# Algorithmic-Alignment-Lab/sco_py

Hardware: AMD Instinct MI355X
Metric: SCO iters/sec (batch of N trajopt QPs) (higher is better)
Workload: dtype f64

## Files before the change

include/sco_hip.h:

```cpp
#ifndef SCO_HIP_H
#define SCO_HIP_H

#ifdef __cplusplus
extern "C" {
#endif

#define SCO_OK              0
#define SCO_ERR_ARG        -1
#define SCO_ERR_DEVICE     -2
#define SCO_ERR_NO_GPU     -3
#define SCO_ERR_STATE      -4
#define SCO_ERR_CAPACITY   -5

#define SCO_QP_SOLVED                 1
#define SCO_QP_SOLVED_INACCURATE      2
#define SCO_QP_MAX_ITER_REACHED      -2
#define SCO_QP_PRIMAL_INFEASIBLE     -3
#define SCO_QP_PRIMAL_INFEASIBLE_INACCURATE 3
#define SCO_QP_DUAL_INFEASIBLE       -4
#define SCO_QP_DUAL_INFEASIBLE_INACCURATE   4
#define SCO_QP_NON_CVX               -7
#define SCO_QP_UNSOLVED             -10

const char *sco_last_error(void);
// ... 159 lines not shown

int sco_sqp_solve(sco_sqp *h, const sco_sqp_params *params, const sco_qp_settings *qp_settings);

int sco_sqp_fetch(sco_sqp *h, double *x, int *success, int *sqp_iters, int *qp_solves,
                  long long *admm_iters, double *merit, double *max_violation);

#define SCO_SQP_FLAG_MEMO_FULL 1
#define SCO_SQP_FLAG_CAPPED 2
#define SCO_SQP_FLAG_TRACE_FULL 4
int sco_sqp_fetch_flags(sco_sqp *h, int *flags);
int sco_sqp_last_rounds(const sco_sqp *h, int *rounds);
int sco_sqp_last_launches(const sco_sqp *h, int *launches, int *groups);

int sco_sqp_last_tiers(const sco_sqp *h, double ms[2], long long iters[2], int launches[2]);

int sco_debug_sqp_mixed(const sco_sqp *h, int out[2]);
int sco_debug_mix_split(int live, int cus, int xcds, int slack, int per_cu);

int sco_debug_wv_gres_slot(int nstep, int pos, int out[5]);

int sco_debug_sqp_schedule(const int in[12], int plan[20], const int round_in[3], int round_out[8]);
int sco_debug_stage_sweep(int n, const double *begin_ms, const double *end_ms, const int *stage, double ms[5]);

int sco_debug_sqp_layout(const sco_trajopt_desc *desc, int n_rows, const int *row_ptr, const int *col_idx, const int *row_is_eq,
                         int dims[22], int sizes[15], int *ints, double *vals);
int sco_debug_sqp_check_program(const sco_trajopt_desc *desc, int n_circle_rows, int n_words, const int *words, const int *row_ptr,
                                int n_consts, int n_params);

int sco_debug_qp_launch_plan(const int *in, const double *tol, int *out);
int sco_debug_plan_tiers(int *mask);

int sco_debug_lanes(int device, int op, const double *a, const double *b, double *out_a, double *out_b);

int sco_sqp_trace(sco_sqp *h, int cap, double *trace, int *n_entries);

int sco_sqp_last_timing(const sco_sqp *h, double ms[5]);

#ifdef __cplusplus
}
#endif
#endif
```

sco_py_amd/_lib.py:

```python
import ctypes as C
import os

import numpy as np

from . import _build

SCO_OK = 0
ERR_NAMES = {-1: "SCO_ERR_ARG", -2: "SCO_ERR_DEVICE", -3: "SCO_ERR_NO_GPU",
             -4: "SCO_ERR_STATE", -5: "SCO_ERR_CAPACITY"}


class ScoHipError(RuntimeError):
    def __init__(self, code, msg):
        super().__init__("%s (%d): %s" % (ERR_NAMES.get(code, "SCO_ERR"), code, msg))
        self.code = code


class QpSettings(C.Structure):
    _fields_ = [
        ("rho", C.c_double), ("sigma", C.c_double), ("alpha", C.c_double),
        ("eps_abs", C.c_double), ("eps_rel", C.c_double),
        ("eps_prim_inf", C.c_double), ("eps_dual_inf", C.c_double),
        ("max_iter", C.c_int), ("check_termination", C.c_int), ("scaling", C.c_int),
        ("warm_start", C.c_int), ("adaptive_rho", C.c_int), ("adaptive_rho_interval", C.c_int),
# ... 54 lines not shown
    "sco_sqp_load_quadratic": (C.c_int, [C.c_void_p, _DP, _DP, _DP]),
    "sco_sqp_load_spatial": (C.c_int, [C.c_void_p, _DP, _DP, _DP, _DP, _DP]),
    "sco_sqp_load_program": (C.c_int, [C.c_void_p, C.c_int, _IP, _IP, C.c_int, _DP, C.c_int, _DP]),
    "sco_sqp_load_program_steps": (C.c_int, [C.c_void_p, C.c_int, _IP, _IP, C.c_int, _DP, C.c_int, _DP]),
    "sco_sqp_load_obj_weights": (C.c_int, [C.c_void_p, _DP]),
    "sco_sqp_load_acc_weights": (C.c_int, [C.c_void_p, _DP]),
    "sco_sqp_load_linear_rows": (C.c_int, [C.c_void_p, _DP, _DP]),
    "sco_sqp_set_circle_rows": (C.c_int, [C.c_void_p, C.c_int]),
    "sco_sqp_load_vel_limit": (C.c_int, [C.c_void_p, _DP]),
    "sco_sqp_load_joint_limits": (C.c_int, [C.c_void_p, _DP, _DP]),
    "sco_sqp_load_ee_cost": (C.c_int, [C.c_void_p, _DP, _DP]),
    "sco_sqp_set_groups": (C.c_int, [C.c_void_p, C.c_int, C.POINTER(C.c_uint)]),
    "sco_sqp_fetch_groups": (C.c_int, [C.c_void_p, C.POINTER(C.c_uint)]),
    "sco_sqp_fetch_stalled_groups": (C.c_int, [C.c_void_p, C.POINTER(C.c_uint)]),
    "sco_sqp_fetch_flags": (C.c_int, [C.c_void_p, _IP]),
    "sco_sqp_last_rounds": (C.c_int, [C.c_void_p, _IP]),
    "sco_sqp_last_launches": (C.c_int, [C.c_void_p, _IP, _IP]),
    "sco_sqp_last_tiers": (C.c_int, [C.c_void_p, _DP, _LP, _IP]),
    "sco_debug_sqp_mixed": (C.c_int, [C.c_void_p, _IP]),
    "sco_debug_mix_split": (C.c_int, [C.c_int, C.c_int, C.c_int, C.c_int, C.c_int]),
    "sco_debug_wv_gres_slot": (C.c_int, [C.c_int, C.c_int, _IP]),
    "sco_debug_sqp_schedule": (C.c_int, [_IP, _IP, _IP, _IP]),
    "sco_debug_stage_sweep": (C.c_int, [C.c_int, _DP, _DP, _IP, _DP]),
    "sco_debug_sqp_layout": (C.c_int, [C.POINTER(TrajoptDesc), C.c_int, _IP, _IP, _IP, _IP, _IP, _IP, _DP]),
    "sco_debug_sqp_check_program": (C.c_int, [C.POINTER(TrajoptDesc), C.c_int, C.c_int, _IP, _IP, C.c_int, C.c_int]),
    "sco_debug_qp_launch_plan": (C.c_int, [_IP, _DP, _IP]),
    "sco_debug_plan_tiers": (C.c_int, [_IP]),
    "sco_debug_lanes": (C.c_int, [C.c_int, C.c_int, _DP, _DP, _DP, _DP]),
    "sco_sqp_solve": (C.c_int, [C.c_void_p, C.POINTER(SqpParams), C.POINTER(QpSettings)]),
    "sco_sqp_fetch": (C.c_int, [C.c_void_p, _DP, _IP, _IP, _IP, _LP, _DP, _DP]),
    "sco_sqp_trace": (C.c_int, [C.c_void_p, C.c_int, _DP, _IP]),
    "sco_sqp_last_timing": (C.c_int, [C.c_void_p, _DP]),
}

_lib = None


def lib_path():
    return _build.LIB


def load():
    global _lib
    if _lib is not None:
        return _lib
    path = lib_path()
# ... 141 lines not shown
```

sco_py_amd/csrc/sco_sqp.hip:

```cpp
#include "sco_admm_check.h"
#include "sqp_layout.h"
#include "sqp_rows.h"
#include "sqp_sched.h"

#include <algorithm>

#include <cmath>
#include <cstdio>
#include <cstdlib>
#include <cstring>

enum { ST_PROJECT = 0, ST_CONVEXIFY = 1, ST_TRIAL = 2, ST_DONE = 3 };
enum { STEP_PROJECT = 0, STEP_ACCEPT = 1, STEP_SHRINK = 2, STEP_YCONV = 3, STEP_XCONV = 4, STEP_BAD = 5, STEP_GROUP = 6 };

#define TRACE_W 8

struct SqpScalars {
  double penalty, trust, slack_cost, merit, merit_viol;
  long long admm_iters;
  int state, k, sqp_iters, qp_solves, success, escalations, n_trace, spawned;
  int flags;
};

struct EventPool {
// ... 42 lines not shown
  int *newqp;
  const int *list;
  int *list_buf;
  const int *jpos;
  const int *epos;
  int G;
  const unsigned int *gmask;
  const unsigned int *goverlap;
  double *mvec;
  unsigned int *nonconv;
  unsigned int *stalled;
  int H, HC;
  double *hkey, *hval, *ckey, *cJ, *cb;
  int *hn, *cn;
};

struct sco_sqp {
  int device = 0;
  sco_trajopt_desc desc{};
  sco_qp *qp0 = nullptr, *qp1 = nullptr;
  SqpDev d{};
  hipStream_t stream = nullptr;
  hipStream_t gstream[SQP_MAX_GROUPS - 1] = {};
  EventPool events, gevents[SQP_MAX_GROUPS];
  EventPool done{{}, 0, hipEventDisableTiming};
  EventPool mix_events{{}, 0, hipEventDisableTiming};
  int xcds = 0;
  double *fetch_buf = nullptr;
  int *host_active = nullptr;
  int groups_used = 1;
  std::vector<void *> allocs;
  void *prog_buf[4] = {nullptr, nullptr, nullptr, nullptr};
  void *objw_buf = nullptr;
  void *accw_buf = nullptr;
  bool gen_loaded = false;
  size_t prog_bytes[4] = {0, 0, 0, 0};
  bool loaded = false, solved = false, target_loaded = false, vel_loaded = false, jl_loaded = false, cost_loaded = false, quad_loaded = false, prog_loaded = false, spatial_loaded = false;
  double last_ms[5] = {0, 0, 0, 0, 0};
  int rounds = 0;
  int launches = 0;
  int wv_rounds = 0;
  double wv_ms = 0.0;
  int mixed_rounds = 0, mixed_side = 0;
};

__device__ __forceinline__ int memo_find(const double *keys, int count, int d, const double *x) {
// ... 264 lines not shown
          }
          wave_lds_fence();
        }
    double lam = A[0];
    for (int i = 1; i < n; i++) lam = fmin(lam, A[i * WIDE_LD + i]);
    if (lane < n) {
      if (lam < 0.0) Ht[lane * n + lane] -= lam;
      const double g = oA[t * n + lane];
      double acc = 0.0;
      for (int i = 0; i < n; i++) acc += th[i] * Ht[i * n + lane];
      xh[lane] = acc; gl[lane] = g;
      oA[t * n + lane] = g - acc;
    }
    wave_lds_fence();
    if (lane == 0) {
      double xHx = 0.0, gx = 0.0;
      for (int j = 0; j < n; j++) { xHx += xh[j] * th[j]; gx += gl[j] * th[j]; }
      ob[t] = (0.5 * xHx - gx) + of0[t];
    }
    wave_lds_fence();
  }
}

template <bool WIDE>
__device__ __forceinline__ void sqp_pre_body(SqpDev &s, QpDev &q1, SqpParamsDev &p) {
  const int g = blockIdx.x + s.b0, tid = threadIdx.x;
  const int b = s.list ? s.list[g] : g;
  if (b < 0) return;
  SqpScalars &sc = s.sc[b];
  const int state = sc.state;
  const bool parked = q1.prog && q1.prog[b] > 0;
  if (tid == 0) s.newqp[b] = (state != ST_DONE && !parked) ? 1 : 0;
  if (state == ST_DONE || parked) return;
  __shared__ double red[NWAVE * 4];
  __shared__ double of0[260];
  const int n_x = s.n_x, d = s.d, T = s.T, R = s.R, n = s.n, m = s.m;
  const int ds = s.ds, NBt = s.NBt;
  const int NO = s.cost == OBJ_BLOCK ? NBt : T;
  const RowLay L{T, NBt, R, s.Req};
  double *x = s.x + (size_t)b * n_x, *xs = s.x_saved + (size_t)b * n_x;
  double *gs = s.gsave + (size_t)b * s.m_nl, *J = s.J + (size_t)b * s.m_nl * ds, *bm = s.bmod + (size_t)b * s.m_nl;
  unsigned char *mask = s.mask + (size_t)b * s.m_nl * ds;
  const double penalty = sc.penalty, trust = sc.trust;
  const int spawned = sc.spawned;
  int k_rows = sc.k;
  double slack_cost = sc.slack_cost;

  if (state == ST_CONVEXIFY) {
    __shared__ int ev_hit[260], cv_hit[260];
    const int H = s.H, HC = s.HC, NB = s.NB, RM = s.RM, m_nl = s.m_nl;
    const RowCtx rc = row_ctx(s, b);
    double *hkey = s.hkey + (size_t)b * NB * H * ds, *hval = s.hval + (size_t)b * NB * H * RM;
    double *ckey = s.ckey + (size_t)b * NB * HC * ds, *cJ = s.cJ + (size_t)b * NB * HC * RM * ds, *cb = s.cb + (size_t)b * NB * HC * RM;
    int *hn = s.hn + (size_t)b * NB, *cn = s.cn + (size_t)b * NB;
    memo_lookup(s, p.memo, hkey, hn, H, x, ev_hit);
    memo_lookup(s, p.memo, ckey, cn, HC, x, cv_hit);
    __syncthreads();
    for (int e = tid; e < m_nl; e += SCO_BLOCK) {
      const RowRef q = row_ref(e, L);
      double g;
      if (ev_hit[q.blk] >= 0) g = hval[((size_t)q.blk * H + ev_hit[q.blk]) * RM + q.r];
      else {
        g = row_value(rc, q, x + q.t * d, -1, 0.0);
        if (p.memo && hn[q.blk] < H) hval[((size_t)q.blk * H + hn[q.blk]) * RM + q.r] = g;
      }
      gs[e] = g;
    }
    for (int e = tid; e < m_nl * ds; e += SCO_BLOCK) {
      const int j = e % ds;
      const RowRef q = row_ref(e / ds, L);
      const double *th = x + q.t * d;
      double val;
      if (q.eq == ROW_REACH_EQ && j >= d) {
        val = 0.0;
      } else if (cv_hit[q.blk] >= 0) {
        val = cJ[(((size_t)q.blk * HC + cv_hit[q.blk]) * RM + q.r) * ds + j];
      } else if (s.analytic_jac) {
        val = row_grad(rc, q, th, j);
      } else if (row_ignores(rc, q, j)) {
        val = 0.0;
      } else {
        val = central_diff(th[j], j, [&](int jj, double h) { return row_value(rc, q, th, jj, h); });
      }
      J[e] = val;
      if (p.memo && cv_hit[q.blk] < 0 && cn[q.blk] < HC) cJ[(((size_t)q.blk * HC + cn[q.blk]) * RM + q.r) * ds + j] = val;
      if (!spawned) mask[e] = (val != 0.0) ? 1 : 0;
    }
    __syncthreads();
    if (p.duplicate_rows) k_rows += 1; else k_rows = 1;
    slack_cost = p.compound_penalty ? slack_cost * penalty : penalty;
    double *Av = q1.Aval + (size_t)b * q1.nnzA;
    double *l = q1.l + (size_t)b * m, *u = q1.u + (size_t)b * m;
    int *w = q1.w + (size_t)b * m;
    for (int e = tid; e < m_nl; e += SCO_BLOCK) {
      const RowRef q = row_ref(e, L);
      double bb = (gs[e] - model_row(J, x, q, e, d, ds)) - row_rhs(rc, q);
      if (cv_hit[q.blk] >= 0) bb = cb[((size_t)q.blk * HC + cv_hit[q.blk]) * RM + q.r];
      else if (p.memo && cn[q.blk] < HC) cb[((size_t)q.blk * HC + cn[q.blk]) * RM + q.r] = bb;
      bm[e] = bb;
      u[s.m_lin + e] = -bb;
      if (q.eq != ROW_HINGE) l[s.m_lin + e] = -bb;
      w[s.m_lin + e] = k_rows;
    }
    for (int e = tid; e < m_nl * ds; e += SCO_BLOCK) {
      const int j = e % ds;
      const RowRef q = row_ref(e / ds, L);
      if (q.eq == ROW_REACH_EQ && j >= d) continue;
      const int c = q.t * d + j, tfirst = (c / d - s.S + 1 > 0) ? c / d - s.S + 1 : 0;
      const int pos = q.eq == ROW_REACH_EQ ? s.epos[j] + q.r : s.jpos[c] + (q.blk - tfirst) * R + q.r;
// ... 364 lines not shown
  s.batch = B; s.d = d; s.T = T; s.K = K; s.O = O; s.R = L.R; s.n_x = n_x; s.n_slack = L.n_slack; s.n = L.n;
  s.m_lin = L.m_lin; s.m_nl = m_nl; s.m = L.m; s.prox_count = desc->prox_count > 0 ? desc->prox_count : 1;
  s.analytic_jac = desc->analytic_jac; s.trace_cap = 64;
  s.point = L.point;
  s.NE = L.NE; s.NB = L.NB; s.RM = L.RM;
  s.S = L.S; s.ds = ds; s.NBt = NBt; s.Req = L.Req;
  s.m_gen = L.m_gen; s.nnz_gen = L.nnz_gen;
  s.acc = L.acc;
  s.m_pin = L.m_pin; s.m_vel = L.m_vel; s.m_jl = L.m_jl; s.cost = L.cost;
#define AL(f, cnt) if ((rc = sq_alloc(h, (cnt), &s.f))) return rc;
  AL(x0, (size_t)B * n_x) AL(start, (size_t)B * d) AL(goal, (size_t)B * d) AL(link_len, (size_t)B * d)
  AL(obstacles, (size_t)B * O * 3) AL(target, (size_t)B * 2) AL(vmax, (size_t)B) AL(jlo, (size_t)B * d) AL(jhi, (size_t)B * d)
  {
    const bool quadf = L.point == ROWS_QUADRATIC;
    AL(qQ, quadf ? (size_t)B * O * ds * ds : 1) AL(qa, quadf ? (size_t)B * O * ds : 1) AL(qc, quadf ? (size_t)B * O : 1)
  }
  {
    const bool spf = L.point == ROWS_SPATIAL;
    AL(sp_off, spf ? (size_t)B * d * 3 : 1) AL(sp_axis, spf ? (size_t)B * d * 3 : 1) AL(sp_pos, spf ? (size_t)B * K * 3 : 1)
    AL(sp_rad, spf ? (size_t)B * K : 1) AL(sp_sph, spf ? (size_t)B * O * 4 : 1)
  }
  AL(x, (size_t)B * n_x) AL(x_saved, (size_t)B * n_x) AL(gsave, (size_t)B * m_nl) AL(J, (size_t)B * m_nl * ds)
  AL(bmod, (size_t)B * m_nl) AL(trace, (size_t)B * s.trace_cap * TRACE_W) AL(mask, (size_t)B * m_nl * ds)
  AL(sc, (size_t)B) AL(active, (size_t)B) AL(n_active, SQP_MAX_GROUPS) AL(newqp, (size_t)B) AL(list_buf, (size_t)B)
  s.H = 40; s.HC = 24;
  AL(hkey, (size_t)B * s.NB * s.H * ds) AL(hval, (size_t)B * s.NB * s.H * s.RM) AL(ckey, (size_t)B * s.NB * s.HC * ds)
  AL(cJ, (size_t)B * s.NB * s.HC * s.RM * ds) AL(cb, (size_t)B * s.NB * s.HC * s.RM) AL(hn, (size_t)B * s.NB)
  AL(cn, (size_t)B * s.NB)
  AL(cw, (size_t)B) AL(ctgt, (size_t)B * 2)
  {
    const size_t NO = oblk ? NBt : T, dO = oblk ? ds : d;
    if (desc->family & SCO_FAM_FLAG_OBJ_WIDE) {
      void *p = nullptr;
      const size_t bytes = (size_t)B * NO * dO * dO * sizeof(double);
      if (hipMalloc(&p, bytes) != hipSuccess) {
        (void)hipGetLastError();
        char buf[200];
        snprintf(buf, sizeof buf, "sco_sqp_create: the objective terms' Hessians (batch x terms x n^2 doubles) need %zu bytes of "
                 "device memory; use a smaller batch", bytes);
        sco_set_error(buf); return SCO_ERR_CAPACITY;
      }
      h->allocs.push_back(p); s.oH = (double *)p;
      SCO_HIP(hipMemset(p, 0, bytes));
    } else {
      AL(oH, cost ? (size_t)B * NO * dO * dO : 1)
    }
    AL(oA, cost ? (size_t)B * NO * dO : 1) AL(ob, cost ? (size_t)B * NO : 1)
// ... 10 lines not shown
  s.gen_eq = s.gpos0 = s.gpos1 = nullptr; s.gen_rhs = s.gen_val = nullptr;
  if (L.m_gen) {
    double *q;
    if ((rc = sq_upload(h, L.gen_eq, &s.gen_eq)) || (rc = sq_upload(h, L.gpos0, &s.gpos0)) || (rc = sq_upload(h, L.gpos1, &s.gpos1))) return rc;
    if ((rc = sq_alloc(h, (size_t)B * L.m_gen, &q))) return rc; s.gen_rhs = q;
    if ((rc = sq_alloc(h, (size_t)B * L.nnz_gen, &q))) return rc; s.gen_val = q;
  }
  return SCO_OK;
}

extern "C" int sco_sqp_destroy(sco_sqp *h) {
  if (!h) return SCO_OK;
  ScoDeviceGuard sco_guard_(h->device);
  if (h->stream) (void)hipStreamSynchronize(h->stream);
  if (h->qp0) sco_qp_destroy(h->qp0);
  if (h->qp1) sco_qp_destroy(h->qp1);
  for (void *p : h->allocs) (void)hipFree(p);
  for (void *p : h->prog_buf) if (p) (void)hipFree(p);
  if (h->objw_buf) (void)hipFree(h->objw_buf);
  if (h->accw_buf) (void)hipFree(h->accw_buf);
  h->events.destroy(); h->done.destroy(); h->mix_events.destroy();
  for (auto &ge : h->gevents) ge.destroy();
  for (auto gs : h->gstream) if (gs) { (void)hipStreamSynchronize(gs); (void)hipStreamDestroy(gs); }
  if (h->host_active) (void)hipHostFree(h->host_active);
  if (h->stream) (void)hipStreamDestroy(h->stream);
  delete h;
  return SCO_OK;
}

extern "C" int sco_sqp_load(sco_sqp *h, const double *x0, const double *start, const double *goal,
                            const double *link_len, const int *point_link, const double *point_frac,
                            const double *obstacles) {
  if (!h || !x0 || !start || !goal || !link_len || !point_link || !point_frac || !obstacles) {
    sco_set_error("sco_sqp_load: null pointer"); return SCO_ERR_ARG;
  }
  const SqpDev &s = h->d;
  for (int k = 0; k < s.K; k++)
    if (point_link[k] < 0 || point_link[k] >= s.d) { sco_set_error("sco_sqp_load: point_link out of range"); return SCO_ERR_ARG; }
  SCO_ON_DEVICE(h->device);
  const size_t B = s.batch;
  SCO_HIP(hipMemcpyAsync(s.x0, x0, B * s.n_x * sizeof(double), hipMemcpyHostToDevice, h->stream));
  SCO_HIP(hipMemcpyAsync(s.start, start, B * s.d * sizeof(double), hipMemcpyHostToDevice, h->stream));
  SCO_HIP(hipMemcpyAsync(s.goal, goal, B * s.d * sizeof(double), hipMemcpyHostToDevice, h->stream));
  SCO_HIP(hipMemcpyAsync(s.link_len, link_len, B * s.d * sizeof(double), hipMemcpyHostToDevice, h->stream));
  SCO_HIP(hipMemcpyAsync(s.obstacles, obstacles, B * s.O * 3 * sizeof(double), hipMemcpyHostToDevice, h->stream));
  SCO_HIP(hipMemcpyAsync((void *)s.point_link, point_link, s.K * sizeof(int), hipMemcpyHostToDevice, h->stream));
// ... 235 lines not shown
  for (size_t b = 0; b < B; b++) flags[b] = sc[b].flags;
  return SCO_OK;
}

extern "C" int sco_sqp_fetch_groups(sco_sqp *h, unsigned int *nonconverged) {
  if (!h || !nonconverged) return SCO_ERR_ARG;
  if (!h->solved) { sco_set_error("sco_sqp_fetch_groups: call sco_sqp_solve first"); return SCO_ERR_STATE; }
  SCO_ON_DEVICE(h->device);
  SCO_HIP(hipMemcpy(nonconverged, h->d.nonconv, (size_t)h->d.batch * sizeof(unsigned int), hipMemcpyDeviceToHost));
  return SCO_OK;
}

extern "C" int sco_sqp_fetch_stalled_groups(sco_sqp *h, unsigned int *stalled) {
  if (!h || !stalled) return SCO_ERR_ARG;
  if (!h->solved) { sco_set_error("sco_sqp_fetch_stalled_groups: call sco_sqp_solve first"); return SCO_ERR_STATE; }
  SCO_ON_DEVICE(h->device);
  SCO_HIP(hipMemcpy(stalled, h->d.stalled, (size_t)h->d.batch * sizeof(unsigned int), hipMemcpyDeviceToHost));
  return SCO_OK;
}

#define SEL_T 1024
#define SEL_BUCKETS 1024
static_assert(SEL_T == SQP_SEL_MAX && SCO_WV_PER_CU == SQP_WV_PER_CU, "sqp_sched.h plans with the kernels' sizes");
__global__ __launch_bounds__(SEL_T) void sqp_select_kernel(SqpDev s, QpDev q1, int cus, int slice, int max_iter, int cap, int nb, int order) {
  __shared__ int hist[SEL_BUCKETS];
  __shared__ int part[SEL_T], part2[SEL_T];
  __shared__ int s_active, s_thr, s_take;
  const int tid = threadIdx.x, B = nb, gb0 = s.b0;
  int *list = s.list_buf + gb0;
  for (int k = tid; k < SEL_BUCKETS; k += SEL_T) hist[k] = 0;
  if (tid == 0) s_active = 0;
  __syncthreads();
  const int per_qp = slice > 0 ? (max_iter + slice - 1) / slice : 1;
  auto key_of = [&](int b) -> int {
    const SqpScalars &sc = s.sc[b];
    if (sc.state == ST_DONE) return -1;
    const int done = (q1.prog && slice > 0) ? q1.prog[b] / slice : 0;
    const int est = max(per_qp - done, 0) + (sc.qp_solves <= 1 ? per_qp : 0);
    return max(SEL_BUCKETS - 1 - est, 0);
  };
  const int per = (B + SEL_T - 1) / SEL_T, b0 = gb0 + min(B, tid * per), b1 = min(gb0 + B, b0 + per);
  int mine = 0;
  for (int b = b0; b < b1; b++) {
    const int k = key_of(b);
    if (k >= 0) { atomicAdd(&hist[k], 1); mine++; }
  }
  if (mine) atomicAdd(&s_active, mine);
  __syncthreads();
  const int A = s_active;
  const int quota = min(cap, (cus <= 0 || A <= cus) ? A : (A / cus) * cus);
  if (tid == 0) {
    int acc = 0, k = 0;
    for (; k < SEL_BUCKETS; k++) { if (acc + hist[k] > quota) break; acc += hist[k]; }
    s_thr = k; s_take = quota - acc;
    *s.n_active = A - quota;
  }
  __syncthreads();
  const int thr = s_thr, take = s_take;
  int cnt = 0;
  for (int b = b0; b < b1; b++) cnt += key_of(b) == thr ? 1 : 0;
  part[tid] = cnt;
  __syncthreads();
  if (tid == 0) { int acc = 0; for (int t = 0; t < SEL_T; t++) { const int v = part[t]; part[t] = acc; acc += v; } }
  __syncthreads();
  int seen = part[tid], chosen = 0;
  for (int b = b0; b < b1; b++) {
    const int k = key_of(b);
    if (k >= 0 && k < thr) chosen++;
    else if (k == thr) { if (seen < take) chosen++; seen++; }
  }
  part2[tid] = chosen;
  __syncthreads();
  if (tid == 0) { int acc = 0; for (int t = 0; t < SEL_T; t++) { const int v = part2[t]; part2[t] = acc; acc += v; } }
  __syncthreads();
  int pos = part2[tid];
  seen = part[tid];
  for (int b = b0; b < b1; b++) {
    const int k = key_of(b);
    bool r = false;
    if (k >= 0 && k < thr) r = true;
    else if (k == thr) { r = seen < take; seen++; }
    if (r) list[pos++] = b;
  }
  for (int g = quota + tid; g < cap; g += SEL_T) list[g] = -1;
  if (order && quota <= SEL_T) {
    __syncthreads();
    const int mine_b = tid < quota ? list[tid] : -1, mine_k = tid < quota ? key_of(mine_b) : SEL_BUCKETS;
    part[tid] = mine_k;
    __syncthreads();
    int rank = 0;
    for (int j = 0; j < quota; j++) { const int kj = part[j]; rank += (kj < mine_k || (kj == mine_k && j < tid)) ? 1 : 0; }
    __syncthreads();
    if (tid < quota) list[rank] = mine_b;
  }
}

__global__ void sqp_cap_kernel(SqpDev s) {
  const int b = blockIdx.x * blockDim.x + threadIdx.x;
  if (b >= s.batch) return;
  SqpScalars &sc = s.sc[b];
  if (sc.state != ST_DONE) { sc.state = ST_DONE; sc.success = 0; sc.flags |= SCO_SQP_FLAG_CAPPED; s.active[b] = 0; }
// ... 109 lines not shown
static SqpSchedule sqp_plan(sco_sqp *h, int admm_slice, const sco_qp_settings &qsl, int max_qp_solves, int n_active) {
  SqpSchedIn in;
  in.batch = h->d.batch;
  (void)hipDeviceGetAttribute(&in.cus, hipDeviceAttributeMultiprocessorCount, h->device);
  in.admm_slice = admm_slice; in.max_qp_solves = max_qp_solves; in.n_active = n_active;
  in.adaptive_rho = qsl.adaptive_rho; in.max_iter = qsl.max_iter;
  in.adaptive_interval = qsl.adaptive_rho ? sco_qp_adaptive_interval(&qsl) : 0;
  in.supports_groups = sco_qp_supports_groups(h->qp1, &qsl);
  in.handle_wv = sco_qp_has_wv(h->qp1) && !(qsl.adaptive_rho && sco_qp_wv_links(h->qp1));
  in.wv_min = sco_wv_min_live(in.cus, qsl.adaptive_rho != 0);
  if (in.handle_wv) {
    if (!h->xcds) h->xcds = sqp_xcds(h->device, in.cus);
    in.xcds = h->xcds;
  }
  in.env = sqp_sched_env();
  return sqp_schedule_plan(in);
}

static int sqp_loop_start(SqpLoop &L) {
  sco_sqp *h = L.h;
  const SqpSchedule &sc = L.sc;
  if (sc.trace) fprintf(stderr, "sco_sqp_solve: %d CUs, %d stream group(s), round selection %s, slice %d\n", sc.cus, sc.G, sc.select ? "on" : "off", sc.slice);
  if (sc.mix_on && !h->gstream[0]) SCO_HIP(hipStreamCreate(&h->gstream[0]));
  h->groups_used = sc.G;
  for (int g = 1; g < sc.G; g++)
    if (!h->gstream[g - 1]) SCO_HIP(hipStreamCreate(&h->gstream[g - 1]));
  for (int g = 0; g < sc.G; g++) {
    SqpGroupRun &r = L.grp[g];
    r.b0 = sc.grp[g].b0; r.nb = sc.grp[g].nb; r.last_active = sc.grp[g].live;
    r.st = g == 0 ? h->stream : h->gstream[g - 1];
    h->gevents[g].rewind();
    r.marks.pool = &h->gevents[g]; r.marks.st = r.st;
  }
  h->done.rewind(); h->mix_events.rewind();
  for (int i = 0; i < sc.G * SQP_DEPTH; i++)
    SCO_TRY(h->done.next(&L.done[i]));
  if (sc.G > 1) {
    hipEvent_t ready;
    SCO_TRY(L.main.take(-2, &ready));
    SCO_HIP(hipEventRecord(ready, h->stream));
    for (int g = 1; g < sc.G; g++) SCO_HIP(hipStreamWaitEvent(L.grp[g].st, ready, 0));
  }
  return SCO_OK;
}

static int sqp_enqueue_round(SqpLoop &L, int g) {
  sco_sqp *h = L.h;
  const SqpSchedule &sc = L.sc;
  const SqpDev &s = h->d;
  SqpGroupRun &r = L.grp[g];
  const SqpRound rp = sqp_round_plan(sc, r.nb, r.last_active, r.issued);
  const dim3 block(SCO_BLOCK);
  SqpDev sg = s; sg.b0 = r.b0; sg.n_active = s.n_active + g;
  if (r.issued == 0) SCO_TRY(r.marks.mark(-1));
  if (!sc.select) SCO_HIP(hipMemsetAsync(sg.n_active, 0, sizeof(int), r.st));
  sg.list = nullptr;
  if (sc.select) {
    hipLaunchKernelGGL(sqp_select_kernel, dim3(1), dim3(SEL_T), 0, r.st, sg, h->qp1->d, rp.pass, sc.slice, L.qsl.max_iter, rp.nwg, r.nb, rp.mix_k > 0 ? 1 : 0);
    SCO_HIP(hipGetLastError());
    sg.list = s.list_buf;
  }
  if (h->desc.family & SCO_FAM_FLAG_OBJ_WIDE)
    hipLaunchKernelGGL(sqp_pre_wide_kernel, dim3(rp.nwg), block, WIDE_LDS_BYTES, r.st, sg, h->qp1->d, L.p);
  else
    hipLaunchKernelGGL(sqp_pre_kernel, dim3(rp.nwg), block, 0, r.st, sg, h->qp1->d, L.p);
  SCO_HIP(hipGetLastError());
  SCO_TRY(r.marks.mark(0));
  hipEvent_t gm;
  SCO_TRY(r.marks.take(1, &gm));
  QpGroup win{r.b0, rp.nwg, r.st, sg.list, rp.tier};
  if (rp.mix_k > 0) {
    win.side_nb = rp.mix_k; win.side_slices = sc.mix_slices; win.side_stream = h->gstream[0];
    win.side_b0 = r.b0 + rp.side_off;
    for (int e = 0; e < 3; e++)
      SCO_TRY(h->mix_events.next(&win.side_ev[e]));
    L.mixed_rounds++; L.mixed_side += rp.mix_k;
  }
  if (g == 0) L.round_k.push_back(rp.mix_k > 0 ? rp.mix_k : (rp.wv_round ? 0 : -1));
  if (rp.counts_as_wv) L.wv_rounds++;
  SCO_TRY(sco_qp_launch_sliced(h->qp1, &L.qsl, s.newqp, s.active, sc.slice, gm, nullptr, rp.window ? &win : nullptr));
  SCO_TRY(r.marks.mark(rp.counts_as_wv ? 5 : 2));
  hipLaunchKernelGGL(sqp_post_kernel, dim3(rp.nwg), block, 0, r.st, sg, h->qp1->d, L.p);
  SCO_HIP(hipGetLastError());
  SCO_TRY(r.marks.mark(3));
  const int slot = r.issued % SQP_DEPTH;
  SCO_HIP(hipMemcpyAsync(h->host_active + g * SQP_DEPTH + slot, sg.n_active, sizeof(int), hipMemcpyDeviceToHost, r.st));
  SCO_HIP(hipEventRecord(L.done[g * SQP_DEPTH + slot], r.st));
  r.issued++;
  return SCO_OK;
}

static void sqp_trace_round(const SqpLoop &L, int g) {
  const SqpGroupRun &r = L.grp[g];
  if (!L.sc.trace || !(r.retired < 40 || r.retired % 100 == 0 || L.sc.trace >= 2)) return;
  const int rk = (g == 0 && L.sc.has_wv) ? L.round_k[r.retired - 1] : -2;
  char kind[48] = "";
  if (rk > 0) snprintf(kind, sizeof kind, " (mixed round, k = %d)", rk);
  else if (rk > -2) snprintf(kind, sizeof kind, rk == 0 ? " (wavefront round)" : " (row-local round)");
  fprintf(stderr, "sco_sqp_solve: group %d round %d, %d problems active%s\n", g, r.retired, r.last_active, kind);
}

static int sqp_run_rounds(SqpLoop &L) {
  const SqpSchedule &sc = L.sc;
  for (int k = 0; k < sc.depth; k++)
    for (int g = 0; g < sc.G; g++)
      SCO_TRY(sqp_enqueue_round(L, g));
  for (bool busy = true; busy;) {
    busy = false;
    for (int g = 0; g < sc.G; g++) {
      SqpGroupRun &r = L.grp[g];
// ... 151 lines not shown
  for (int k = 0; k < 13; k++) {
    sizes[k] = (int)iv[k]->size();
    if (ints) ints = std::copy(iv[k]->begin(), iv[k]->end(), ints);
  }
  for (int k = 0; k < 2; k++) {
    sizes[13 + k] = (int)dv[k]->size();
    if (vals) vals = std::copy(dv[k]->begin(), dv[k]->end(), vals);
  }
  return SCO_OK;
}
extern "C" int sco_debug_sqp_check_program(const sco_trajopt_desc *desc, int n_circle_rows, int n_words, const int *words,
                                           const int *row_ptr, int n_consts, int n_params) {
  const char *err = "";
  if (int rc = sqp_check_desc(desc, 0, nullptr, nullptr, nullptr, &err)) { sco_set_error(err); return rc; }
  if (!words || !row_ptr) { sco_set_error("sco_sqp_load_program: null pointer"); return SCO_ERR_ARG; }
  if ((desc->family & 15) != SCO_FAM_STATE_PROGRAM) { sco_set_error("sco_sqp_load_program: family has no row programs"); return SCO_ERR_ARG; }
  const SqpLayout L = sqp_layout_build(*desc, 0, nullptr, nullptr, nullptr);
  if (n_circle_rows < 0 || n_circle_rows >= desc->n_obstacles) { sco_set_error("sco_debug_sqp_check_program: bad circle-row count"); return SCO_ERR_ARG; }
  const int rc = sqp_check_program(desc->n_obstacles - n_circle_rows, L.cost, L.ds, desc->dof, n_words, words, row_ptr, n_consts, n_params, &err);
  if (rc) sco_set_error(err);
  return rc;
}

extern "C" int sco_debug_sqp_wv_rounds(const sco_sqp *h) { return h ? h->wv_rounds : -1; }
extern "C" int sco_debug_sqp_mixed(const sco_sqp *h, int out[2]) {
  if (!h || !out) return SCO_ERR_ARG;
  out[0] = h->mixed_rounds; out[1] = h->mixed_side;
  return SCO_OK;
}
extern "C" int sco_sqp_last_tiers(const sco_sqp *h, double ms[2], long long iters[2], int launches[2]) {
  if (!h || !ms || !iters || !launches) return SCO_ERR_ARG;
  SCO_ON_DEVICE(h->device);
  unsigned long long wv_it = 0;
  if (sco_qp_wv_iters(h->qp1, &wv_it)) return SCO_ERR_DEVICE;
  ms[0] = h->wv_ms; ms[1] = h->last_ms[2] - h->wv_ms;
  iters[0] = (long long)wv_it; iters[1] = -1;
  launches[0] = h->wv_rounds; launches[1] = h->launches - h->wv_rounds + h->mixed_rounds;
  return SCO_OK;
}
extern "C" int sco_sqp_last_launches(const sco_sqp *h, int *launches, int *groups) {
  if (!h) return SCO_ERR_ARG;
  if (launches) *launches = h->launches;
  if (groups) *groups = h->groups_used;
  return SCO_OK;
}

// ... 6 lines not shown
```

sco_py_amd/csrc/sqp_sched.cpp:

```cpp
#include "sqp_sched.h"

#include <algorithm>
#include <climits>
#include <cstdlib>
#include <cstring>
#include <vector>

SqpSchedEnv sqp_sched_env() {
  SqpSchedEnv e;
  auto env_int = [](const char *name, int dflt) { const char *v = getenv(name); return v ? atoi(v) : dflt; };
  e.slice = std::max(0, env_int("SCO_SQP_SLICE", 0));
  e.groups = env_int("SCO_SQP_GROUPS", 1);
  { const char *v = getenv("SCO_SQP_SELECT"); e.select = !(v && v[0] == '0'); }
  e.mix = env_int("SCO_SQP_MIX", SQP_MIX_DEFAULT);
  e.mix_slack = env_int("SCO_SQP_MIX_SLACK", 1);
  e.mix_slices = env_int("SCO_SQP_MIX_SLICES", 2);
  { const char *v = getenv("SCO_SQP_MIX_PICK"); e.mix_tail = v && !strcmp(v, "tail"); }
  e.xcds = std::max(0, env_int("SCO_SQP_XCDS", 0));
  { const char *v = getenv("SCO_SQP_TRACE_ROUNDS"); e.trace = !v ? 0 : (atoi(v) >= 2 ? 2 : 1); }
  return e;
}

SqpSchedule sqp_schedule_plan(const SqpSchedIn &in) {
  SqpSchedule sc;
  sc.cus = in.cus; sc.wv_min = in.wv_min; sc.handle_wv = in.handle_wv; sc.trace = in.env.trace;
  const int batch = in.batch, cus = in.cus;
  int slice = in.admm_slice < 0 ? 0 : (in.admm_slice > 0 ? in.admm_slice : (in.adaptive_rho ? 2000 : 6250));
  if (in.admm_slice == 0) {
    if (in.env.slice > 0) slice = in.env.slice;
    if (cus > 0 && batch <= cus) slice = 0;
  }
  sc.slice = slice;
  long long slices_per_qp = slice > 0 ? (in.max_iter + slice - 1) / slice : 1;
  if (in.adaptive_rho) slices_per_qp += in.max_iter / in.adaptive_interval + 1;
  sc.round_cap = 2 * ((long long)in.max_qp_solves + 8) * slices_per_qp;
  if (slice > 0 && in.supports_groups && cus > 0 && batch >= 2 * cus)
    sc.G = std::max(1, std::min(std::min(in.env.groups, SQP_MAX_GROUPS), batch / cus));
  sc.select = slice > 0 && cus > 0 && batch > cus && in.supports_groups && in.env.select;
  sc.has_wv = sc.select && in.handle_wv;
  sc.mix_on = sc.has_wv && sc.G == 1 && !in.adaptive_rho && in.env.mix != 0;
  sc.mix_slack = std::max(0, in.env.mix_slack); sc.mix_slices = std::max(1, in.env.mix_slices);
  sc.xcds = sc.mix_on ? (in.env.xcds > 0 ? in.env.xcds : in.xcds) : 1;
  sc.mix_tail = in.env.mix_tail;
  sc.depth = (!sc.select && sc.G == 1 && slice == 0) ? 1 : SQP_DEPTH;
  for (int g = 0; g < sc.G; g++) {
    sc.grp[g].b0 = (int)((long long)batch * g / sc.G); sc.grp[g].nb = (int)((long long)batch * (g + 1) / sc.G) - sc.grp[g].b0;
    sc.grp[g].live = sc.G == 1 ? in.n_active : sc.grp[g].nb;
  }
// ... 85 lines not shown
```

sco_py_amd/csrc/sqp_sched.h:

```cpp
#pragma once

#define SQP_MAX_GROUPS 4
#define SQP_DEPTH 2
#define SQP_MIX_DEFAULT 1
#define SQP_WV_PER_CU 4
#define SQP_SEL_MAX 1024

struct SqpSchedEnv {
  int slice = 0;
  int groups = 1;
  bool select = true;
  int mix = SQP_MIX_DEFAULT;
  int mix_slack = 1;
  int mix_slices = 2;
  bool mix_tail = false;
  int xcds = 0;
  int trace = 0;
};
SqpSchedEnv sqp_sched_env();

struct SqpSchedIn {
  int batch = 0, cus = 0;
  int admm_slice = 0;
  int adaptive_rho = 0, max_iter = 0, adaptive_interval = 0;
  int max_qp_solves = 0;
  int n_active = 0;
  bool supports_groups = false;
  bool handle_wv = false;
  int wv_min = 0;
  int xcds = 1;
  SqpSchedEnv env;
};

struct SqpSchedule {
  int cus = 0;
  int slice = 0;
  int G = 1;
  struct { int b0, nb, live; } grp[SQP_MAX_GROUPS] = {};
  bool select = false;
  bool has_wv = false, handle_wv = false;
  int wv_min = 0;
  bool mix_on = false, mix_tail = false;
  int mix_slack = 0, mix_slices = 1, xcds = 1;
  int depth = SQP_DEPTH;
  long long round_cap = 0;
  int trace = 0;
};
SqpSchedule sqp_schedule_plan(const SqpSchedIn &in);

struct SqpRound {
  bool wv_round = false;
  int pass = 0;
  int nwg = 0;
  int mix_k = 0;
  int side_off = 0;
  int tier = 0;
  bool window = false;
  bool counts_as_wv = false;
};
SqpRound sqp_round_plan(const SqpSchedule &sc, int group_nb, int live, int round_index);

int qp_mix_split(int live, int cus, int xcds, int slack, int per_cu);

void sqp_stage_sweep(const double *begin_ms, const double *end_ms, const int *stage, int n, double ms[5]);
```

Before: 6981.

## Split Jacobian into multi-block kernel, parallel-scan selection, async copy stream

Moves the Jacobian/finite-difference computation out of the per-problem pre kernel into a separate kernel that uses a 2D grid, so several blocks share each problem's Jacobian entries. Replaces the single-thread serial prefix sums in the round-selection kernel with a wave-shuffle block scan, and caches the first key per thread. Double-buffers the n_active counter per depth slot and issues the device-to-host copy on a dedicated copy stream when there is one group. It also adds a debug entry point for the selection kernel. The extra kernel launch and duplicated memo lookup add overhead that may offset the gains.

After: 7047, median of 6. About the same (+0.9%).

```diff
diff --git a/include/sco_hip.h b/include/sco_hip.h
--- a/include/sco_hip.h
+++ b/include/sco_hip.h
@@ -205,6 +205,9 @@
 int sco_debug_sqp_schedule(const int in[12], int plan[20], const int round_in[3], int round_out[8]);
 int sco_debug_stage_sweep(int n, const double *begin_ms, const double *end_ms, const int *stage, double ms[5]);
 
+int sco_debug_sqp_select(int device, int nb, const int *done, const int *qp_solves, const int *prog, int cus, int slice,
+                         int max_iter, int cap, int order, int *list, int *left);
+
 int sco_debug_sqp_layout(const sco_trajopt_desc *desc, int n_rows, const int *row_ptr, const int *col_idx, const int *row_is_eq,
                          int dims[22], int sizes[15], int *ints, double *vals);
 int sco_debug_sqp_check_program(const sco_trajopt_desc *desc, int n_circle_rows, int n_words, const int *words, const int *row_ptr,
diff --git a/sco_py_amd/_lib.py b/sco_py_amd/_lib.py
--- a/sco_py_amd/_lib.py
+++ b/sco_py_amd/_lib.py
@@ -100,6 +100,7 @@
     "sco_debug_wv_gres_slot": (C.c_int, [C.c_int, C.c_int, _IP]),
     "sco_debug_sqp_schedule": (C.c_int, [_IP, _IP, _IP, _IP]),
     "sco_debug_stage_sweep": (C.c_int, [C.c_int, _DP, _DP, _IP, _DP]),
+    "sco_debug_sqp_select": (C.c_int, [C.c_int, C.c_int, _IP, _IP, _IP, C.c_int, C.c_int, C.c_int, C.c_int, C.c_int, _IP, _IP]),
     "sco_debug_sqp_layout": (C.c_int, [C.POINTER(TrajoptDesc), C.c_int, _IP, _IP, _IP, _IP, _IP, _IP, _DP]),
     "sco_debug_sqp_check_program": (C.c_int, [C.POINTER(TrajoptDesc), C.c_int, C.c_int, _IP, _IP, C.c_int, C.c_int]),
     "sco_debug_qp_launch_plan": (C.c_int, [_IP, _DP, _IP]),
diff --git a/sco_py_amd/csrc/sco_sqp.hip b/sco_py_amd/csrc/sco_sqp.hip
--- a/sco_py_amd/csrc/sco_sqp.hip
+++ b/sco_py_amd/csrc/sco_sqp.hip
@@ -88,6 +88,7 @@
   SqpDev d{};
   hipStream_t stream = nullptr;
   hipStream_t gstream[SQP_MAX_GROUPS - 1] = {};
+  hipStream_t copy_stream = nullptr;
   EventPool events, gevents[SQP_MAX_GROUPS];
   EventPool done{{}, 0, hipEventDisableTiming};
   EventPool mix_events{{}, 0, hipEventDisableTiming};
@@ -398,6 +399,48 @@
   }
 }
 
+#define SQP_JAC_SPLIT_MAX 8
+__global__ __launch_bounds__(SCO_BLOCK) void sqp_jac_kernel(SqpDev s, QpDev q1, SqpParamsDev p) {
+  const int g = blockIdx.x + s.b0, tid = threadIdx.x;
+  const int b = s.list ? s.list[g] : g;
+  if (b < 0) return;
+  const SqpScalars &sc = s.sc[b];
+  if (sc.state != ST_CONVEXIFY || (q1.prog && q1.prog[b] > 0)) return;
+  __shared__ int cv_hit[260];
+  const int d = s.d, ds = s.ds, HC = s.HC, NB = s.NB, RM = s.RM, m_nl = s.m_nl;
+  const RowLay L{s.T, s.NBt, s.R, s.Req};
+  const double *x = s.x + (size_t)b * s.n_x;
+  double *J = s.J + (size_t)b * m_nl * ds;
+  unsigned char *mask = s.mask + (size_t)b * m_nl * ds;
+  const int spawned = sc.spawned;
+  const RowCtx rc = row_ctx(s, b);
+  const double *ckey = s.ckey + (size_t)b * NB * HC * ds;
+  double *cJ = s.cJ + (size_t)b * NB * HC * RM * ds;
+  const int *cn = s.cn + (size_t)b * NB;
+  memo_lookup(s, p.memo, ckey, cn, HC, x, cv_hit);
+  __syncthreads();
+  for (int e = blockIdx.y * SCO_BLOCK + tid; e < m_nl * ds; e += gridDim.y * SCO_BLOCK) {
+    const int j = e % ds;
+    const RowRef q = row_ref(e / ds, L);
+    const double *th = x + q.t * d;
+    double val;
+    if (q.eq == ROW_REACH_EQ && j >= d) {
+      val = 0.0;
+    } else if (cv_hit[q.blk] >= 0) {
+      val = cJ[(((size_t)q.blk * HC + cv_hit[q.blk]) * RM + q.r) * ds + j];
+    } else if (s.analytic_jac) {
+      val = row_grad(rc, q, th, j);
+    } else if (row_ignores(rc, q, j)) {
+      val = 0.0;
+    } else {
+      val = central_diff(th[j], j, [&](int jj, double h) { return row_value(rc, q, th, jj, h); });
+    }
+    J[e] = val;
+    if (p.memo && cv_hit[q.blk] < 0 && cn[q.blk] < HC) cJ[(((size_t)q.blk * HC + cn[q.blk]) * RM + q.r) * ds + j] = val;
+    if (!spawned) mask[e] = (val != 0.0) ? 1 : 0;
+  }
+}
+
 template <bool WIDE>
 __device__ __forceinline__ void sqp_pre_body(SqpDev &s, QpDev &q1, SqpParamsDev &p) {
   const int g = blockIdx.x + s.b0, tid = threadIdx.x;
@@ -418,7 +461,6 @@
   double *gs = s.gsave + (size_t)b * s.m_nl, *J = s.J + (size_t)b * s.m_nl * ds, *bm = s.bmod + (size_t)b * s.m_nl;
   unsigned char *mask = s.mask + (size_t)b * s.m_nl * ds;
   const double penalty = sc.penalty, trust = sc.trust;
-  const int spawned = sc.spawned;
   int k_rows = sc.k;
   double slack_cost = sc.slack_cost;
 
@@ -427,7 +469,7 @@
     const int H = s.H, HC = s.HC, NB = s.NB, RM = s.RM, m_nl = s.m_nl;
     const RowCtx rc = row_ctx(s, b);
     double *hkey = s.hkey + (size_t)b * NB * H * ds, *hval = s.hval + (size_t)b * NB * H * RM;
-    double *ckey = s.ckey + (size_t)b * NB * HC * ds, *cJ = s.cJ + (size_t)b * NB * HC * RM * ds, *cb = s.cb + (size_t)b * NB * HC * RM;
+    double *ckey = s.ckey + (size_t)b * NB * HC * ds, *cb = s.cb + (size_t)b * NB * HC * RM;
     int *hn = s.hn + (size_t)b * NB, *cn = s.cn + (size_t)b * NB;
     memo_lookup(s, p.memo, hkey, hn, H, x, ev_hit);
     memo_lookup(s, p.memo, ckey, cn, HC, x, cv_hit);
@@ -441,26 +483,6 @@
         if (p.memo && hn[q.blk] < H) hval[((size_t)q.blk * H + hn[q.blk]) * RM + q.r] = g;
       }
       gs[e] = g;
-    }
-    for (int e = tid; e < m_nl * ds; e += SCO_BLOCK) {
-      const int j = e % ds;
-      const RowRef q = row_ref(e / ds, L);
-      const double *th = x + q.t * d;
-      double val;
-      if (q.eq == ROW_REACH_EQ && j >= d) {
-        val = 0.0;
-      } else if (cv_hit[q.blk] >= 0) {
-        val = cJ[(((size_t)q.blk * HC + cv_hit[q.blk]) * RM + q.r) * ds + j];
-      } else if (s.analytic_jac) {
-        val = row_grad(rc, q, th, j);
-      } else if (row_ignores(rc, q, j)) {
-        val = 0.0;
-      } else {
-        val = central_diff(th[j], j, [&](int jj, double h) { return row_value(rc, q, th, jj, h); });
-      }
-      J[e] = val;
-      if (p.memo && cv_hit[q.blk] < 0 && cn[q.blk] < HC) cJ[(((size_t)q.blk * HC + cn[q.blk]) * RM + q.r) * ds + j] = val;
-      if (!spawned) mask[e] = (val != 0.0) ? 1 : 0;
     }
     __syncthreads();
     if (p.duplicate_rows) k_rows += 1; else k_rows = 1;
@@ -871,7 +893,7 @@
   }
   AL(x, (size_t)B * n_x) AL(x_saved, (size_t)B * n_x) AL(gsave, (size_t)B * m_nl) AL(J, (size_t)B * m_nl * ds)
   AL(bmod, (size_t)B * m_nl) AL(trace, (size_t)B * s.trace_cap * TRACE_W) AL(mask, (size_t)B * m_nl * ds)
-  AL(sc, (size_t)B) AL(active, (size_t)B) AL(n_active, SQP_MAX_GROUPS) AL(newqp, (size_t)B) AL(list_buf, (size_t)B)
+  AL(sc, (size_t)B) AL(active, (size_t)B) AL(n_active, SQP_MAX_GROUPS * SQP_DEPTH) AL(newqp, (size_t)B) AL(list_buf, (size_t)B)
   s.H = 40; s.HC = 24;
   AL(hkey, (size_t)B * s.NB * s.H * ds) AL(hval, (size_t)B * s.NB * s.H * s.RM) AL(ckey, (size_t)B * s.NB * s.HC * ds)
   AL(cJ, (size_t)B * s.NB * s.HC * s.RM * ds) AL(cb, (size_t)B * s.NB * s.HC * s.RM) AL(hn, (size_t)B * s.NB)
@@ -928,6 +950,7 @@
   h->events.destroy(); h->done.destroy(); h->mix_events.destroy();
   for (auto &ge : h->gevents) ge.destroy();
   for (auto gs : h->gstream) if (gs) { (void)hipStreamSynchronize(gs); (void)hipStreamDestroy(gs); }
+  if (h->copy_stream) { (void)hipStreamSynchronize(h->copy_stream); (void)hipStreamDestroy(h->copy_stream); }
   if (h->host_active) (void)hipHostFree(h->host_active);
   if (h->stream) (void)hipStreamDestroy(h->stream);
   delete h;
@@ -1209,9 +1232,23 @@
 #define SEL_T 1024
 #define SEL_BUCKETS 1024
 static_assert(SEL_T == SQP_SEL_MAX && SCO_WV_PER_CU == SQP_WV_PER_CU, "sqp_sched.h plans with the kernels' sizes");
+static_assert(SEL_BUCKETS == SEL_T && SEL_T % 64 == 0, "sqp_select_kernel scans the buckets one per thread");
+__device__ __forceinline__ int sel_scan(int v, int *wsum, int *total) {
+  const int lane = threadIdx.x & 63, w = threadIdx.x >> 6;
+  int incl = v;
+#pragma unroll
+  for (int o = 1; o < 64; o <<= 1) { const int up = __shfl_up(incl, o); if (lane >= o) incl += up; }
+  __syncthreads();
+  if (lane == 63) wsum[w] = incl;
+  __syncthreads();
+  int off = 0, all = 0;
+  for (int k = 0; k < SEL_T / 64; k++) { const int sum = wsum[k]; off += k < w ? sum : 0; all += sum; }
+  if (total) *total = all;
+  return off + incl - v;
+}
 __global__ __launch_bounds__(SEL_T) void sqp_select_kernel(SqpDev s, QpDev q1, int cus, int slice, int max_iter, int cap, int nb, int order) {
   __shared__ int hist[SEL_BUCKETS];
-  __shared__ int part[SEL_T], part2[SEL_T];
+  __shared__ int part[SEL_T], wsum[SEL_T / 64];
   __shared__ int s_active, s_thr, s_take;
   const int tid = threadIdx.x, B = nb, gb0 = s.b0;
   int *list = s.list_buf + gb0;
@@ -1227,43 +1264,41 @@
     return max(SEL_BUCKETS - 1 - est, 0);
   };
   const int per = (B + SEL_T - 1) / SEL_T, b0 = gb0 + min(B, tid * per), b1 = min(gb0 + B, b0 + per);
+  const int key_first = b0 < b1 ? key_of(b0) : -1;
+  auto key_at = [&](int b) -> int { return b == b0 ? key_first : key_of(b); };
   int mine = 0;
   for (int b = b0; b < b1; b++) {
-    const int k = key_of(b);
+    const int k = key_at(b);
     if (k >= 0) { atomicAdd(&hist[k], 1); mine++; }
   }
   if (mine) atomicAdd(&s_active, mine);
   __syncthreads();
   const int A = s_active;
   const int quota = min(cap, (cus <= 0 || A <= cus) ? A : (A / cus) * cus);
-  if (tid == 0) {
-    int acc = 0, k = 0;
-    for (; k < SEL_BUCKETS; k++) { if (acc + hist[k] > quota) break; acc += hist[k]; }
-    s_thr = k; s_take = quota - acc;
-    *s.n_active = A - quota;
+  {
+    int all = 0;
+    const int own = hist[tid], front = sel_scan(own, wsum, &all);
+    if (front <= quota && front + own > quota) { s_thr = tid; s_take = quota - front; }
+    if (tid == 0) {
+      if (all <= quota) { s_thr = SEL_BUCKETS; s_take = quota - all; }
+      *s.n_active = A - quota;
+    }
   }
   __syncthreads();
   const int thr = s_thr, take = s_take;
   int cnt = 0;
-  for (int b = b0; b < b1; b++) cnt += key_of(b) == thr ? 1 : 0;
-  part[tid] = cnt;
-  __syncthreads();
-  if (tid == 0) { int acc = 0; for (int t = 0; t < SEL_T; t++) { const int v = part[t]; part[t] = acc; acc += v; } }
-  __syncthreads();
-  int seen = part[tid], chosen = 0;
+  for (int b = b0; b < b1; b++) cnt += key_at(b) == thr ? 1 : 0;
+  const int seen0 = sel_scan(cnt, wsum, nullptr);
+  int seen = seen0, chosen = 0;
   for (int b = b0; b < b1; b++) {
-    const int k = key_of(b);
+    const int k = key_at(b);
     if (k >= 0 && k < thr) chosen++;
     else if (k == thr) { if (seen < take) chosen++; seen++; }
   }
-  part2[tid] = chosen;
-  __syncthreads();
-  if (tid == 0) { int acc = 0; for (int t = 0; t < SEL_T; t++) { const int v = part2[t]; part2[t] = acc; acc += v; } }
-  __syncthreads();
-  int pos = part2[tid];
-  seen = part[tid];
+  int pos = sel_scan(chosen, wsum, nullptr);
+  seen = seen0;
   for (int b = b0; b < b1; b++) {
-    const int k = key_of(b);
+    const int k = key_at(b);
     bool r = false;
     if (k >= 0 && k < thr) r = true;
     else if (k == thr) { r = seen < take; seen++; }
@@ -1419,6 +1454,7 @@
   const SqpSchedule &sc = L.sc;
   if (sc.trace) fprintf(stderr, "sco_sqp_solve: %d CUs, %d stream group(s), round selection %s, slice %d\n", sc.cus, sc.G, sc.select ? "on" : "off", sc.slice);
   if (sc.mix_on && !h->gstream[0]) SCO_HIP(hipStreamCreate(&h->gstream[0]));
+  if (!h->copy_stream) SCO_HIP(hipStreamCreate(&h->copy_stream));
   h->groups_used = sc.G;
   for (int g = 1; g < sc.G; g++)
     if (!h->gstream[g - 1]) SCO_HIP(hipStreamCreate(&h->gstream[g - 1]));
@@ -1448,7 +1484,8 @@
   SqpGroupRun &r = L.grp[g];
   const SqpRound rp = sqp_round_plan(sc, r.nb, r.last_active, r.issued);
   const dim3 block(SCO_BLOCK);
-  SqpDev sg = s; sg.b0 = r.b0; sg.n_active = s.n_active + g;
+  const int slot = r.issued % SQP_DEPTH;
+  SqpDev sg = s; sg.b0 = r.b0; sg.n_active = s.n_active + g * SQP_DEPTH + slot;
   if (r.issued == 0) SCO_TRY(r.marks.mark(-1));
   if (!sc.select) SCO_HIP(hipMemsetAsync(sg.n_active, 0, sizeof(int), r.st));
   sg.list = nullptr;
@@ -1456,6 +1493,11 @@
     hipLaunchKernelGGL(sqp_select_kernel, dim3(1), dim3(SEL_T), 0, r.st, sg, h->qp1->d, rp.pass, sc.slice, L.qsl.max_iter, rp.nwg, r.nb, rp.mix_k > 0 ? 1 : 0);
     SCO_HIP(hipGetLastError());
     sg.list = s.list_buf;
+  }
+  {
+    const int jac_split = std::max(1, std::min(SQP_JAC_SPLIT_MAX, sc.jac_split > 0 ? sc.jac_split : (s.m_nl * s.ds + SCO_BLOCK - 1) / SCO_BLOCK));
+    hipLaunchKernelGGL(sqp_jac_kernel, dim3(rp.nwg, jac_split), block, 0, r.st, sg, h->qp1->d, L.p);
+    SCO_HIP(hipGetLastError());
   }
   if (h->desc.family & SCO_FAM_FLAG_OBJ_WIDE)
     hipLaunchKernelGGL(sqp_pre_wide_kernel, dim3(rp.nwg), block, WIDE_LDS_BYTES, r.st, sg, h->qp1->d, L.p);
@@ -1479,10 +1521,13 @@
   SCO_TRY(r.marks.mark(rp.counts_as_wv ? 5 : 2));
   hipLaunchKernelGGL(sqp_post_kernel, dim3(rp.nwg), block, 0, r.st, sg, h->qp1->d, L.p);
   SCO_HIP(hipGetLastError());
-  SCO_TRY(r.marks.mark(3));
-  const int slot = r.issued % SQP_DEPTH;
-  SCO_HIP(hipMemcpyAsync(h->host_active + g * SQP_DEPTH + slot, sg.n_active, sizeof(int), hipMemcpyDeviceToHost, r.st));
-  SCO_HIP(hipEventRecord(L.done[g * SQP_DEPTH + slot], r.st));
+  hipEvent_t decided;
+  SCO_TRY(r.marks.take(3, &decided));
+  SCO_HIP(hipEventRecord(decided, r.st));
+  hipStream_t cs = sc.G == 1 ? h->copy_stream : r.st;
+  if (cs != r.st) SCO_HIP(hipStreamWaitEvent(cs, decided, 0));
+  SCO_HIP(hipMemcpyAsync(h->host_active + g * SQP_DEPTH + slot, sg.n_active, sizeof(int), hipMemcpyDeviceToHost, cs));
+  SCO_HIP(hipEventRecord(L.done[g * SQP_DEPTH + slot], cs));
   r.issued++;
   return SCO_OK;
 }
@@ -1680,6 +1725,35 @@
   return rc;
 }
 
+extern "C" int sco_debug_sqp_select(int device, int nb, const int *done, const int *qp_solves, const int *prog, int cus, int slice,
+                                    int max_iter, int cap, int order, int *list, int *left_out) {
+  if (nb <= 0 || cap <= 0 || cap > nb || slice < 0 || max_iter <= 0 || !done || !qp_solves || !prog || !list || !left_out) {
+    sco_set_error("sco_debug_sqp_select: bad argument (0 < cap <= nb, slice >= 0, max_iter > 0, no null pointer)"); return SCO_ERR_ARG;
+  }
+  SCO_ON_DEVICE(device);
+  std::vector<void *> allocs;
+  SqpDev s{}; QpDev q1{};
+  int rc = [&]() -> int {
+    std::vector<SqpScalars> sc((size_t)nb, SqpScalars{});
+    for (int b = 0; b < nb; b++) { sc[b].state = done[b] ? ST_DONE : ST_TRIAL; sc[b].qp_solves = qp_solves[b]; }
+    SCO_TRY(sco_alloc_zeroed(allocs, (size_t)nb, &s.sc));
+    SCO_TRY(sco_alloc_zeroed(allocs, (size_t)nb, &q1.prog));
+    SCO_TRY(sco_alloc_zeroed(allocs, (size_t)nb, &s.list_buf));
+    SCO_TRY(sco_alloc_zeroed(allocs, (size_t)1, &s.n_active));
+    SCO_HIP(hipMemcpy(s.sc, sc.data(), (size_t)nb * sizeof(SqpScalars), hipMemcpyHostToDevice));
+    SCO_HIP(hipMemcpy(q1.prog, prog, (size_t)nb * sizeof(int), hipMemcpyHostToDevice));
+    s.batch = nb;
+    hipLaunchKernelGGL(sqp_select_kernel, dim3(1), dim3(SEL_T), 0, nullptr, s, q1, cus, slice, max_iter, cap, nb, order ? 1 : 0);
+    SCO_HIP(hipGetLastError());
+    SCO_HIP(hipDeviceSynchronize());
+    SCO_HIP(hipMemcpy(list, s.list_buf, (size_t)cap * sizeof(int), hipMemcpyDeviceToHost));
+    SCO_HIP(hipMemcpy(left_out, s.n_active, sizeof(int), hipMemcpyDeviceToHost));
+    return SCO_OK;
+  }();
+  for (void *p : allocs) (void)hipFree(p);
+  return rc;
+}
+
 extern "C" int sco_debug_sqp_wv_rounds(const sco_sqp *h) { return h ? h->wv_rounds : -1; }
 extern "C" int sco_debug_sqp_mixed(const sco_sqp *h, int out[2]) {
   if (!h || !out) return SCO_ERR_ARG;
diff --git a/sco_py_amd/csrc/sqp_sched.cpp b/sco_py_amd/csrc/sqp_sched.cpp
--- a/sco_py_amd/csrc/sqp_sched.cpp
+++ b/sco_py_amd/csrc/sqp_sched.cpp
@@ -18,12 +18,13 @@
   { const char *v = getenv("SCO_SQP_MIX_PICK"); e.mix_tail = v && !strcmp(v, "tail"); }
   e.xcds = std::max(0, env_int("SCO_SQP_XCDS", 0));
   { const char *v = getenv("SCO_SQP_TRACE_ROUNDS"); e.trace = !v ? 0 : (atoi(v) >= 2 ? 2 : 1); }
+  e.jac_split = std::max(0, env_int("SCO_SQP_JAC_SPLIT", 0));
   return e;
 }
 
 SqpSchedule sqp_schedule_plan(const SqpSchedIn &in) {
   SqpSchedule sc;
-  sc.cus = in.cus; sc.wv_min = in.wv_min; sc.handle_wv = in.handle_wv; sc.trace = in.env.trace;
+  sc.cus = in.cus; sc.wv_min = in.wv_min; sc.handle_wv = in.handle_wv; sc.trace = in.env.trace; sc.jac_split = in.env.jac_split;
   const int batch = in.batch, cus = in.cus;
   int slice = in.admm_slice < 0 ? 0 : (in.admm_slice > 0 ? in.admm_slice : (in.adaptive_rho ? 2000 : 6250));
   if (in.admm_slice == 0) {
diff --git a/sco_py_amd/csrc/sqp_sched.h b/sco_py_amd/csrc/sqp_sched.h
--- a/sco_py_amd/csrc/sqp_sched.h
+++ b/sco_py_amd/csrc/sqp_sched.h
@@ -16,6 +16,7 @@
   bool mix_tail = false;
   int xcds = 0;
   int trace = 0;
+  int jac_split = 0;
 };
 SqpSchedEnv sqp_sched_env();
 
@@ -45,6 +46,7 @@
   int depth = SQP_DEPTH;
   long long round_cap = 0;
   int trace = 0;
+  int jac_split = 0;
 };
 SqpSchedule sqp_schedule_plan(const SqpSchedIn &in);
 
```
